# DerekGloudemans/3D-playground

Hardware: AMD Instinct MI355X
Metric: training images/sec at 1920x1080, ResNet-50 3D-RetinaNet (higher is better)
Workload: dtype f32; 1 GPU; resnet50 directional 3D-RetinaNet, 1920x1080 synthetic frames, batch 8 per GPU, 10 GT boxes/image, fp32, fwd+loss+bwd+clip+Adam (BASELINE configs[1]); global_batch=8, parallelism=dp1

## Files before the change

3d-playground_amd/csrc/conv_igemm_mf16.hip:

```cpp
#include <type_traits>

#include "conv_igemm_tile.h"
#include "conv_wgrad_geom.h"

typedef float f32x4a __attribute__((ext_vector_type(4)));

#ifndef RN_MF16_STG
#define RN_MF16_STG 1
#endif
#ifndef RN_MF16_PF
#define RN_MF16_PF 1
#endif
#ifndef RN_MF16_KO
#define RN_MF16_KO 0
#endif

#define RN_SPLIT_MFMA16(ACC, A, B)                                                        \
    do {                                                                                  \
        ACC = __builtin_amdgcn_mfma_f32_16x16x32_bf16((A).l, (B).h, ACC, 0, 0, 0);        \
        ACC = __builtin_amdgcn_mfma_f32_16x16x32_bf16((A).h, (B).l, ACC, 0, 0, 0);        \
        ACC = __builtin_amdgcn_mfma_f32_16x16x32_bf16((A).m, (B).m, ACC, 0, 0, 0);        \
        ACC = __builtin_amdgcn_mfma_f32_16x16x32_bf16((A).m, (B).h, ACC, 0, 0, 0);        \
        ACC = __builtin_amdgcn_mfma_f32_16x16x32_bf16((A).h, (B).m, ACC, 0, 0, 0);        \
        ACC = __builtin_amdgcn_mfma_f32_16x16x32_bf16((A).h, (B).h, ACC, 0, 0, 0);        \
    } while (0)

template <bool GENERAL, bool RAW, int TERMS, bool STG, int WV = 4>
__device__ __forceinline__ void conv_mf16_tile(const rn_conv_desc &d, const float *__restrict__ x, const float *__restrict__ w,
                                               float *__restrict__ y, const float *__restrict__ scale,
                                               const float *__restrict__ shift, const float *__restrict__ add,
                                               const float *__restrict__ mask, const float *__restrict__ add2, const int tile) {
    constexpr int BK = 32, BM = 32 * WV, BN = 128, NSN = BN / 16;
    constexpr int SR = WV == 8 ? 8 : 16;
    constexpr bool HALF = TERMS == 2;
    constexpr int REC = 32 * TERMS, EB = 2 * TERMS;
    constexpr int BPL = BN * 16;
    constexpr int BSTEP = TERMS * BPL;
    constexpr int NBI = TERMS * BN / 16, IB = NBI / WV;
    constexpr int LDT = BN + 4;
    constexpr int LDSF = 2 * BSTEP > WV * SR * LDT ? 2 * BSTEP : WV * SR * LDT;
    static_assert(NBI % WV == 0 && (WV == 4 || WV == 8) && (TERMS == 2 || TERMS == 3), "tile shape");
    __shared__ float lds[LDSF];

    const int tid = threadIdx.x, lane = tid & 63, wave = tid >> 6;
    const int lr = lane & 15, lg = lane >> 4;
    const int wave_u = __builtin_amdgcn_readfirstlane(wave);
    const int ntn = (d.Cout + BN - 1) / BN;
    const int m0 = (tile / ntn) * BM, n0 = (tile % ntn) * BN;
    const int HoWo = d.Ho * d.Wo;
    const int64_t M = (int64_t)d.N * HoWo;
    const int K = d.kh * d.kw * d.Cin;
    const int Kpad = (K + 31) / 32 * 32;
    const int nks = Kpad / BK;

    const int n_first = (int)(m0 / HoWo);
    const int64_t x_floats = ((int64_t)d.N - 1 - n_first) * d.x_batch_stride + (int64_t)d.Hi * d.Wi * d.Cin;
    const __amdgpu_buffer_rsrc_t rs_a = __builtin_amdgcn_make_buffer_rsrc(
        const_cast<float *>(x + (int64_t)n_first * d.x_batch_stride), (short)0,
        (int)(unsigned)(x_floats * 4 > 0x7FFFFFFF ? 0x7FFFFFFF : x_floats * 4), 0x00020000);
    const v4i32 rs_b = make_rsrc(reinterpret_cast<const char *>(w) + (int64_t)n_first * d.w_batch_stride * EB,
                                 (unsigned)((int64_t)d.Cout * Kpad * EB));
    __shared__ float row_unscale[HALF ? BM : 1];
    float a_scale[2] = {1.f, 1.f};

    unsigned a_mask[2];
    int a_base[2];
    int a_n[2] = {-1, -1}, a_rem[2] = {0, 0};
    __shared__ __attribute__((aligned(16))) char a_stage[STG ? WV * Mf16AGeom::WAVE_BYTES : 16];
    __shared__ int4 row_tab[STG ? BM : 1];
    unsigned s_mask[4] = {0u, 0u, 0u, 0u};
    int s_base[4] = {0, 0, 0, 0};
    auto row_geom = [&](int row, unsigned &mk, int &base, int &n_abs, int &rem_) {
        int a_h = -(1 << 28), a_w = 0, a_img = 0;
        n_abs = -1; rem_ = 0;
        if ((int64_t)m0 + row < M) {
            const unsigned rel = (unsigned)(m0 - n_first * HoWo + row);
            const unsigned n = rel / (unsigned)HoWo;
            const unsigned rem = rel - n * (unsigned)HoWo;
            const unsigned oh = rem / (unsigned)d.Wo, ow = rem - oh * (unsigned)d.Wo;
            a_img = (int)((int64_t)n * d.x_batch_stride * 4);
            a_h = (int)oh * d.a + d.p;
            a_w = (int)ow * d.a + d.p_w;
            n_abs = n_first + (int)n; rem_ = (int)rem;
        }
        mk = 0;
        for (int r = 0, t = 0; r < d.kh; ++r)
            for (int s_ = 0; s_ < d.kw; ++s_, ++t) {
                const int ih = a_h + r * d.b, iw = a_w + s_ * d.b;
                mk |= (unsigned)(((ih | iw) >= 0) & (ih < d.Hi) & (iw < d.Wi)) << t;
            }
        base = a_img + (a_h * d.Wi + a_w) * d.Cin * 4;
    };
    if constexpr (STG) {
        if (tid < BM) {
            unsigned mk; int base, n_abs, rem_;
            row_geom(tid, mk, base, n_abs, rem_);
            row_tab[tid] = make_int4(base, (int)mk, n_abs, rem_);
        }
        __syncthreads();
#pragma unroll
        for (int j = 0; j < 4; ++j) {
            const int4 e = row_tab[32 * wave + Mf16AGeom::dma_row(lane, j)];
            s_base[j] = e.x + 16 * Mf16AGeom::dma_chunk(lane, j);
            s_mask[j] = (unsigned)e.y;
        }
#pragma unroll
        for (int sm = 0; sm < 2; ++sm) {
            const int4 e = row_tab[32 * wave + 16 * sm + lr];
            a_n[sm] = e.z; a_rem[sm] = e.w;
            a_mask[sm] = 0u; a_base[sm] = 0;
        }
    } else {
#pragma unroll
        for (int sm = 0; sm < 2; ++sm) {
            row_geom(32 * wave + 16 * sm + lr, a_mask[sm], a_base[sm], a_n[sm], a_rem[sm]);
            a_base[sm] += 8 * lg * 4;
        }
    }
    int f_r = 0, f_s = 0, f_c = 0;
    typedef float f32x4v __attribute__((ext_vector_type(4)));
    struct ARegs { f32x4v v[4]; };
    auto load_a = [&](ARegs &ar) {
#if RN_MF16_KO & 2
        if (f_c >= 0) { f_c += BK; return; }
#endif
        const int t = f_r * d.kw + f_s;
        const int delta = (f_r * d.Wi + f_s) * d.b * d.Cin * 4;
#pragma unroll
        for (int sm = 0; sm < 2; ++sm) {
            const unsigned valid = 0u - ((a_mask[sm] >> (t & 31)) & 1u);
            const unsigned v = ((unsigned)(a_base[sm] + delta) & valid) | (0x80000000u & ~valid);
            ar.v[2 * sm] = __builtin_bit_cast(f32x4v, __builtin_amdgcn_raw_buffer_load_b128(rs_a, (int)v, f_c * 4, 0));
            ar.v[2 * sm + 1] = __builtin_bit_cast(f32x4v, __builtin_amdgcn_raw_buffer_load_b128(rs_a, (int)(v + 16u), f_c * 4, 0));
        }
        f_c += BK;
        const bool wrap = f_c >= d.Cin;
        f_c = wrap ? 0 : f_c;
        f_s += wrap ? 1 : 0;
        const bool wrap_s = f_s == d.kw;
        f_s = wrap_s ? 0 : f_s;
        f_r += wrap_s ? 1 : 0;
    };

    const v4i32 rs_a4 = make_rsrc(x + (int64_t)n_first * d.x_batch_stride, (unsigned)(x_floats * 4 > 0x7FFFFFFF ? 0x7FFFFFFF : x_floats * 4));
    const unsigned a_lds0 = lds_addr(a_stage) + (unsigned)__builtin_amdgcn_readfirstlane(wave) * Mf16AGeom::WAVE_BYTES;
    auto dma_a = [&]() {
#if RN_MF16_KO & 2
        if (f_c >= 0) { f_c += BK; return; }
#endif
        const int t = f_r * d.kw + f_s;
        const int delta = (f_r * d.Wi + f_s) * d.b * d.Cin * 4;
        const unsigned soff = (unsigned)__builtin_amdgcn_readfirstlane(f_c * 4);
#pragma unroll
        for (int j = 0; j < 4; ++j) {
            const unsigned valid = 0u - ((s_mask[j] >> (t & 31)) & 1u);
            dma16(rs_a4, a_lds0 + 1024u * j, ((unsigned)(s_base[j] + delta) & valid) | (0x80000000u & ~valid), soff);
        }
        f_c += BK;
        const bool wrap = f_c >= d.Cin;
        f_c = wrap ? 0 : f_c;
        f_s += wrap ? 1 : 0;
        const bool wrap_s = f_s == d.kw;
        f_s = wrap_s ? 0 : f_s;
        f_r += wrap_s ? 1 : 0;
    };
    const char *a_rd = a_stage + wave * Mf16AGeom::WAVE_BYTES;
    const int a_ra[2][2] = {{Mf16AGeom::read_addr(lane, 0, 0), Mf16AGeom::read_addr(lane, 0, 1)},
                            {Mf16AGeom::read_addr(lane, 1, 0), Mf16AGeom::read_addr(lane, 1, 1)}};
    auto read_a = [&](ARegs &ar) {
#pragma unroll
        for (int sm = 0; sm < 2; ++sm) {
            ar.v[2 * sm] = *reinterpret_cast<const f32x4v *>(a_rd + a_ra[sm][0]);
            ar.v[2 * sm + 1] = *reinterpret_cast<const f32x4v *>(a_rd + a_ra[sm][1]);
        }
    };

    unsigned b_voff[IB];
#pragma unroll
    for (int j = 0; j < IB; ++j) {
        const int q = wave * IB + j, plane = q / (BN / 16), brow = (q % (BN / 16)) * 16 + (lane >> 2);
        const int c = Mf16Geom::dma_chunk(lane);
        const int n = n0 + brow;
        b_voff[j] = n < d.Cout ? (unsigned)(n * Kpad * EB + (c >> 1) * REC + plane * 32 + (c & 1) * 16) : 0x80000000u;
    }
    const unsigned lds0 = lds_addr(lds);
    auto dma_b = [&](int ks, int buf) {
#if RN_MF16_KO & 8
        if (ks > 0) return;
#endif
#pragma unroll
        for (int j = 0; j < IB; ++j)
            dma16(rs_b, lds0 + (unsigned)(buf * BSTEP * 4 + (wave_u * IB + j) * 1024), b_voff[j], (unsigned)(ks * 2 * REC));
    };

    f32x4a acc[2][NSN];
#pragma unroll
    for (int i = 0; i < 2; ++i)
#pragma unroll
        for (int j = 0; j < NSN; ++j) acc[i][j] = f32x4a{0.f, 0.f, 0.f, 0.f};
    const int fb0 = Mf16Geom::read_addr(lane, 0) / 4;

    constexpr int PF = RN_MF16_PF;
    static_assert(!STG || PF == 1, "staged activations: one step in flight");
    ARegs ar[PF] = {};
    if constexpr (STG) dma_a(); else load_a(ar[0]);
    dma_b(0, 0);
#pragma unroll
    for (int i = 1; i < PF; ++i) load_a(ar[i]);
    if constexpr (HALF) {
        int e[2];
        if (d.x_amax_row_stride == 0) {
            const unsigned char *tb = reinterpret_cast<const unsigned char *>(d.x_amax);
            e[0] = rn_amax_exp_lanes(a_n[0] < 0 ? nullptr : tb + (int64_t)a_n[0] * d.x_amax_img_stride * RN_AMAX_BYTES);
            e[1] = __ballot(a_n[1] != a_n[0]) == 0ull ? e[0]
                 : rn_amax_exp_lanes(a_n[1] < 0 ? nullptr : tb + (int64_t)a_n[1] * d.x_amax_img_stride * RN_AMAX_BYTES);
        } else {
#pragma unroll
            for (int sm = 0; sm < 2; ++sm)
                e[sm] = a_n[sm] < 0 ? 0 : (int)((reinterpret_cast<const unsigned *>(d.x_amax)[(int64_t)a_rem[sm] * d.x_amax_row_stride] >> 23) & 0xffu);
        }
#pragma unroll
        for (int sm = 0; sm < 2; ++sm) {
            const int se = rn_f16_scale_exp_of(e[sm]);
            a_scale[sm] = rn_exp_to_float(se);
            if (lg == 0) row_unscale[32 * wave + 16 * sm + lr] = rn_exp_to_float(254 - se);
        }
    }
    constexpr int CPR = BN / 4, RPI = 64 / CPR;
    const int c4 = lane % CPR;
    const int col = n0 + 4 * c4;
    const bool col_ok = col < d.Cout;
    const bool vec = true;
    const int ncol = 4;
    rn_wait_but<4 * (PF - 1)>();
    __syncthreads();
    auto k_step = [&](int ks, int rb, ARegs &cur) {
        if constexpr (STG) read_a(cur);
        asm volatile("" : "+v"(cur.v[0]), "+v"(cur.v[1]), "+v"(cur.v[2]), "+v"(cur.v[3]));
        typename std::conditional<HALF, SplitH8, Split8>::type sa[2];
#if RN_MF16_KO & 1
#pragma unroll
        for (int q = 0; q < 4; ++q) acc[q & 1][q >> 1] += cur.v[q];
        dma_b(ks + 1, rb ^ 1);
        if constexpr (STG) { asm volatile("s_waitcnt lgkmcnt(0)" ::: "memory"); dma_a(); } else load_a(cur);
        rn_wait_dma();
        __syncthreads();
        if (ks >= 0) return;
#endif
#pragma unroll
        for (int sm = 0; sm < 2; ++sm) {
            const float av[8] = {cur.v[2 * sm][0], cur.v[2 * sm][1], cur.v[2 * sm][2], cur.v[2 * sm][3],
                                 cur.v[2 * sm + 1][0], cur.v[2 * sm + 1][1], cur.v[2 * sm + 1][2], cur.v[2 * sm + 1][3]};
            if constexpr (HALF) sa[sm] = split8h(av, a_scale[sm]);
            else sa[sm] = split8(av);
        }
        dma_b(ks + 1, rb ^ 1);
        if constexpr (STG) {
            asm volatile("s_waitcnt lgkmcnt(0)" ::: "memory");
            dma_a();
        } else load_a(cur);
        const float *S = lds + rb * BSTEP + fb0;
#pragma unroll
        for (int sn = 0; sn < NSN; ++sn) {
            if constexpr (HALF) {
                SplitH8 sb;
                sb.h = *reinterpret_cast<const f16x8 *>(S + 256 * sn);
                sb.l = *reinterpret_cast<const f16x8 *>(S + 256 * sn + BPL);
#pragma unroll
                for (int sm = 0; sm < 2; ++sm) RN_SPLITH_MFMA16(acc[sm][sn], sa[sm], sb);
            } else {
                Split8 sb;
                sb.h = *reinterpret_cast<const bf16x8 *>(S + 256 * sn);
                sb.m = *reinterpret_cast<const bf16x8 *>(S + 256 * sn + BPL);
                sb.l = *reinterpret_cast<const bf16x8 *>(S + 256 * sn + 2 * BPL);
#pragma unroll
                for (int sm = 0; sm < 2; ++sm) RN_SPLIT_MFMA16(acc[sm][sn], sa[sm], sb);
            }
        }
        RN_PIN();
        rn_wait_but<4 * (PF - 1)>();
        __syncthreads();
    };
    constexpr int UN = PF > 2 ? PF : 2;
    for (int ks = 0; ks < nks; ks += UN) {
#pragma unroll
        for (int u = 0; u < UN; ++u)
            if (u == 0 || ks + u < nks) k_step(ks + u, u & 1, ar[u % PF]);
    }

    float *T = lds + wave * (SR * LDT);
    float sc[4] = {1.f, 1.f, 1.f, 1.f}, sh[4] = {0.f, 0.f, 0.f, 0.f};
#pragma unroll
    for (int j = 0; j < 4; ++j) {
        if (!RAW && col_ok && scale != nullptr) sc[j] = scale[col + j];
        if (!RAW && col_ok && shift != nullptr) sh[j] = shift[col + j];
        if (HALF && col_ok) sc[j] *= d.w_unscale[(d.w_batch_stride != 0 ? (int64_t)n_first * d.Cout : 0) + col + j];
    }
    float rn_am = 0.f;
    const int64_t m_last = (int64_t)m0 + BM - 1 < M ? (int64_t)m0 + BM - 1 : M - 1;
    const bool rn_span = (int)(m0 / HoWo) != (int)(m_last / HoWo);
#pragma unroll
    for (int smh = 0; smh < 2 * (16 / SR); ++smh) {
        const int sm = smh / (16 / SR), hp = smh % (16 / SR);
        if (SR == 16 || (lg >> 1) == hp) {
#pragma unroll
            for (int sn = 0; sn < NSN; ++sn)
#pragma unroll
                for (int e = 0; e < 4; ++e) T[(4 * lg + e - hp * SR) * LDT + 16 * sn + lr] = acc[sm][sn][e];
        }
        __builtin_amdgcn_fence(__ATOMIC_RELEASE, "wavefront");
        __builtin_amdgcn_wave_barrier();
        __builtin_amdgcn_fence(__ATOMIC_ACQUIRE, "wavefront");
        constexpr int NIT = SR / RPI, G = 4;
        if (col_ok) {
#pragma unroll 1
            for (int g = 0; g < NIT; g += G) {
                int64_t off_[G];
                float4 mk_[G], ad_[G];
#pragma unroll
                for (int i = 0; i < G; ++i) {
                    const int64_t mr = (int64_t)m0 + 32 * wave + 16 * sm + hp * SR + lane / CPR + RPI * (g + i);
                    const int64_t m = mr < M ? mr : M - 1;
                    RN_EPI_ADDR(GENERAL)
                    off_[i] = off;
                    mk_[i] = make_float4(1.f, 1.f, 1.f, 1.f);
                    ad_[i] = make_float4(0.f, 0.f, 0.f, 0.f);
                    if (!RAW && d.mask_mode != 0) mk_[i] = rn_mask_load4(mask, off, (d.mask_mode & RN_MASK_BITS) != 0);
                    if (!RAW && d.add_mode != 0) ad_[i] = *reinterpret_cast<const float4 *>(add + aoff);
                    (void)a2off;
                }
#pragma unroll
                for (int i = 0; i < G; ++i) {
                    const int r = lane / CPR + RPI * (g + i);
                    const int64_t m = (int64_t)m0 + 32 * wave + 16 * sm + hp * SR + r;
                    if (m < M) {
                        float4 t = *reinterpret_cast<const float4 *>(T + r * LDT + 4 * c4);
                        if constexpr (HALF) { const float ru = row_unscale[32 * wave + 16 * sm + hp * SR + r]; t.x *= ru; t.y *= ru; t.z *= ru; t.w *= ru; }
                        const int64_t off = off_[i];
                        float mk[4] = {mk_[i].x, mk_[i].y, mk_[i].z, mk_[i].w}, ad[4] = {ad_[i].x, ad_[i].y, ad_[i].z, ad_[i].w};
                        if (!RAW && d.add2_mode == 3) {
                            int64_t a2;
                            { RN_EPI_ADDR(GENERAL) a2 = a2off; (void)aoff; (void)off; }
                            if (a2 >= 0) { const float4 q = *reinterpret_cast<const float4 *>(add2 + a2); ad[0] += q.x; ad[1] += q.y; ad[2] += q.z; ad[3] += q.w; }
                        }
#if RN_MF16_KO & 4
                        if (t.x != 1.2345f) continue;
#endif
                        if (RAW) *reinterpret_cast<float4 *>(y + off) = HALF ? make_float4(t.x * sc[0], t.y * sc[1], t.z * sc[2], t.w * sc[3]) : t;
                        else { RN_EPI_FINISH() }
                    }
                }
            }
        }
        __builtin_amdgcn_fence(__ATOMIC_RELEASE, "wavefront");
        __builtin_amdgcn_wave_barrier();
    }
    if (!RAW && !rn_span) rn_amax_note(d.y_amax, m0 / HoWo, rn_am);
}

#ifndef RN_MF16H_OCC
#define RN_MF16H_OCC 3
#endif
template <bool GENERAL, bool RAW, int TERMS, bool STG, int WV = 4>
__global__ __launch_bounds__(64 * WV, WV == 8 ? 2 : (TERMS == 2 ? RN_MF16H_OCC : 3)) void conv_igemm_mf16_kernel(const rn_conv_desc d, const float *__restrict__ x,
                                                              const float *__restrict__ w, float *__restrict__ y,
                                                              const float *__restrict__ scale, const float *__restrict__ shift,
                                                              const float *__restrict__ add, const float *__restrict__ mask,
                                                              const float *__restrict__ add2) {
    conv_mf16_tile<GENERAL, RAW, TERMS, STG, WV>(d, x, w, y, scale, shift, add, mask, add2, xcd_remap(blockIdx.x, gridDim.x));
}

template <int TERMS>
__global__ __launch_bounds__(256, TERMS == 2 ? RN_MF16H_OCC : 3) void conv_igemm_mf16_grouped_kernel(const rn_conv_group g, const float *__restrict__ w,
                                                                      const float *__restrict__ scale,
                                                                      const float *__restrict__ shift) {
    const int tile = xcd_remap(blockIdx.x, gridDim.x);
    int p = 0;
#pragma unroll
    for (int i = 0; i < RN_MAX_GROUP - 1; ++i) p += (i + 1 < g.n && tile >= g.tile_end[i]) ? 1 : 0;
    rn_conv_desc d = g.d[0];
    const float *x = g.x[0], *add = g.add[0], *mask = g.mask[0];
    float *y = g.y[0];
    int first = 0;
#pragma unroll
    for (int i = 1; i < RN_MAX_GROUP; ++i)
        if (p == i) { d = g.d[i]; x = g.x[i]; y = g.y[i]; add = g.add[i]; mask = g.mask[i]; first = g.tile_end[i - 1]; }
    conv_mf16_tile<true, false, TERMS, TERMS == 2 && RN_MF16_STG != 0>(d, x, w, y, scale, shift, add, mask, nullptr, tile - first);
}

static int mf16_on() { return rn_get_option(RN_OPT_MF16); }
static int mf16_min_tiles() { return rn_get_option(RN_OPT_MF16_MIN); }
static bool mf16_geom_ok(const rn_conv_desc *d) {
    return (d->Cin % 32) == 0 && d->div_shift == 0 && d->kh * d->kw <= 24 && (d->Cout % 4) == 0 && d->Cout > 64 && !d->in_relu;
}
static bool mf16_ok(const rn_conv_desc *d) {
    if (!mf16_on() || !mf16_geom_ok(d)) return false;
    if (d->w_format == 3) return d->x_amax != nullptr && d->w_unscale != nullptr;
    return d->w_format == 1;
}
static int64_t mf16_tiles(const rn_conv_desc *d) {
    const int64_t M = (int64_t)d->N * d->Ho * d->Wo;
    return ((M + 127) / 128) * ((d->Cout + 127) / 128);
}

extern "C" int rn_conv_igemm_wants_f16(const rn_conv_desc *d) {
    return rn_get_fp32_mfma() == RN_FP32_SPLIT3 && d->w_batch_stride >= 0;
}

bool rn_igemm_mf16_launch(int variant, const rn_conv_desc *d, const float *x, const float *w, float *y, const float *scale,
                          const float *shift, const float *add, const float *mask, const float *add2, hipStream_t s, int *rc) {
    if (!mf16_ok(d) || (variant != 0 && variant != 4 && variant != 5)) return false;
    const int64_t tiles = mf16_tiles(d);
    const int64_t M_rows = (int64_t)d->N * d->Ho * d->Wo;
    if (tiles < mf16_min_tiles() || tiles > 0x7fffffff) return false;
    const dim3 grid((unsigned)tiles), block(256);
#define RN_MF16_LAUNCH(G, R, T, S) hipLaunchKernelGGL((conv_igemm_mf16_kernel<G, R, T, S>), grid, block, 0, s, *d, x, w, y, scale, shift, add, mask, add2)
    if (d->w_format == 3) {
        static const int stg_min_k = [] { const char *e = getenv("RN_MF16_STG_MIN_K"); return e ? atoi(e) : 256; }();
        const bool stg = RN_MF16_STG != 0 && d->kh * d->kw * d->Cin >= stg_min_k;
        static const int wv8_min = [] { const char *e = getenv("RN_MF16_WV8_MIN"); return e ? atoi(e) : 1; }();
        const int64_t tiles8 = ((M_rows + 255) / 256) * ((d->Cout + 127) / 128);
        if (stg && wv8_min > 0 && d->w_batch_stride == 0 && tiles8 >= wv8_min && tiles8 <= 0x7fffffff) {
            const dim3 grid8((unsigned)tiles8), block8(512);
#define RN_MF16_LAUNCH8(G, R) hipLaunchKernelGGL((conv_igemm_mf16_kernel<G, R, 2, true, 8>), grid8, block8, 0, s, *d, x, w, y, scale, shift, add, mask, add2)
            if (variant == 0) RN_MF16_LAUNCH8(false, true);
            else if (variant == 4) RN_MF16_LAUNCH8(false, false);
            else RN_MF16_LAUNCH8(true, false);
#undef RN_MF16_LAUNCH8
        } else
        if (variant == 0) { if (stg) RN_MF16_LAUNCH(false, true, 2, true); else RN_MF16_LAUNCH(false, true, 2, false); }
        else if (variant == 4) { if (stg) RN_MF16_LAUNCH(false, false, 2, true); else RN_MF16_LAUNCH(false, false, 2, false); }
        else { if (stg) RN_MF16_LAUNCH(true, false, 2, true); else RN_MF16_LAUNCH(true, false, 2, false); }
    } else {
        if (variant == 0) RN_MF16_LAUNCH(false, true, 3, false);
        else if (variant == 4) RN_MF16_LAUNCH(false, false, 3, false);
        else RN_MF16_LAUNCH(true, false, 3, false);
    }
#undef RN_MF16_LAUNCH
    const hipError_t e = hipGetLastError();
    *rc = e == hipSuccess ? RN_OK : (int)e;
    return true;
}

bool rn_igemm_mf16_grouped_launch(const rn_conv_group *g, const float *w, const float *scale, const float *shift, hipStream_t s, int *rc) {
    for (int i = 0; i < g->n; ++i)
        if (!mf16_ok(&g->d[i]) || g->d[i].w_format != g->d[0].w_format) return false;
    rn_conv_group gb = *g;
    int64_t total = 0;
    for (int i = 0; i < g->n; ++i) {
        total += mf16_tiles(&g->d[i]);
        gb.tile_end[i] = (int)total;
    }
    for (int i = g->n; i < RN_MAX_GROUP; ++i) gb.tile_end[i] = (int)total;
    if (total < mf16_min_tiles() || total > 0x7fffffff) return false;
    if (g->d[0].w_format == 3) hipLaunchKernelGGL(conv_igemm_mf16_grouped_kernel<2>, dim3((unsigned)total), dim3(256), 0, s, gb, w, scale, shift);
    else hipLaunchKernelGGL(conv_igemm_mf16_grouped_kernel<3>, dim3((unsigned)total), dim3(256), 0, s, gb, w, scale, shift);
    const hipError_t e = hipGetLastError();
    *rc = e == hipSuccess ? RN_OK : (int)e;
    return true;
}
```

3d-playground_amd/csrc/elementwise.hip:

```cpp
#include "common.h"
#include "mfma_split.h"

__global__ void pack_weights_kernel(const float *__restrict__ src, float *__restrict__ dst, int Cout, int Cin, int kh, int kw,
                                    int kw_pad, int c_pad, int mode, const float *__restrict__ scale, int rows, int Kpad,
                                    int r0, int nr, int s0, int ns) {
    const int64_t i = (int64_t)blockIdx.x * 256 + threadIdx.x;
    if (i >= (int64_t)rows * Kpad) return;
    const int row = (int)(i / Kpad), k = (int)(i - (int64_t)row * Kpad);
    const int tap = k / c_pad, c = k - tap * c_pad;
    int r = tap / kw_pad, s = tap - r * kw_pad;
    bool in_filter = r < kh && s < kw;
    if (mode == 2) {
        r = tap / ns;
        s = tap - r * ns;
        in_filter = r < nr;
        r = r0 + 2 * r;
        s = s0 + 2 * s;
    }
    float v = 0.f;
    if (in_filter) {
        if (mode == 0) {
            if (c < Cin) v = src[(((int64_t)row * Cin + c) * kh + r) * kw + s];
        } else {
            if (c < Cout) {
                v = src[(((int64_t)c * Cin + row) * kh + r) * kw + s];
                if (scale) v *= scale[c];
            }
        }
    }
    dst[i] = v;
}

extern "C" int rn_pack_weights(const float *src, float *dst, int Cout, int Cin, int kh, int kw, int kw_pad, int c_pad,
                               int mode, const float *scale, int r0, int nr, int s0, int ns, void *stream) {
    if (Cout <= 0 || Cin <= 0 || kh <= 0 || kw <= 0 || kw_pad < kw || (c_pad & 3) || mode < 0 || mode > 2) return RN_EINVAL;
    if (c_pad < (mode == 0 ? Cin : Cout)) return RN_EINVAL;
    if (mode == 2 && (nr <= 0 || ns <= 0 || r0 < 0 || s0 < 0 || r0 + 2 * (nr - 1) >= kh || s0 + 2 * (ns - 1) >= kw))
        return RN_EINVAL;
    const int rows = mode == 0 ? Cout : Cin;
    const int Kpad = ((mode == 2 ? nr * ns : kh * kw_pad) * c_pad + 31) / 32 * 32;
    hipLaunchKernelGGL(pack_weights_kernel, dim3(rn_blocks((int64_t)rows * Kpad, 256)), dim3(256), 0, (hipStream_t)stream, src,
                       dst, Cout, Cin, kh, kw, kw_pad, c_pad, mode, scale, rows, Kpad, r0, nr, s0, ns);
    RN_LAUNCH_CHECK();
    return RN_OK;
}

__device__ __forceinline__ void unpack_wgrad_channel(const int co, const float *__restrict__ dw, const float *__restrict__ wp,
                                                     float *__restrict__ dweight, int Cin, int kh, int kw, int kw_pad,
                                                     int c_pad, int Kpad, const float *__restrict__ scale,
                                                     const float *__restrict__ mean, const float *__restrict__ rstd,
                                                     const float *__restrict__ colsum, float *__restrict__ dgamma,
                                                     float *__restrict__ dbeta) {
    __shared__ double red[4];
    const float sc = scale ? scale[co] : 1.f;
    const float *row = dw + (int64_t)co * Kpad;
    const float *wrow = wp + (int64_t)co * Kpad;
    const int n = Cin * kh * kw;
    double dot = 0.0;
    for (int i = threadIdx.x; i < n; i += 256) {
        const int ci = i / (kh * kw), rs = i - ci * (kh * kw);
        const int r = rs / kw, s = rs - r * kw;
        const int k = (r * kw_pad + s) * c_pad + ci;
        const float g = row[k];
        dweight[(int64_t)co * n + i] = sc * g;
        if (dgamma) dot += (double)wrow[k] * (double)g;
    }
    if (dgamma) {
        dot = wave_sum(dot);
        if ((threadIdx.x & 63) == 0) red[threadIdx.x >> 6] = dot;
        __syncthreads();
        if (threadIdx.x == 0) {
            const double t = (red[0] + red[1]) + (red[2] + red[3]);
            dgamma[co] = (float)((t - (double)mean[co] * (double)colsum[co]) * (double)rstd[co]);
        }
    }
    if (dbeta && threadIdx.x == 0) dbeta[co] = colsum[co];
}

__global__ __launch_bounds__(256) void unpack_wgrad_kernel(const float *__restrict__ dw, const float *__restrict__ wp,
                                                           float *__restrict__ dweight, int Cin, int kh, int kw, int kw_pad,
                                                           int c_pad, int Kpad, const float *__restrict__ scale,
                                                           const float *__restrict__ mean, const float *__restrict__ rstd,
                                                           const float *__restrict__ colsum, float *__restrict__ dgamma,
                                                           float *__restrict__ dbeta) {
    unpack_wgrad_channel(blockIdx.x, dw, wp, dweight, Cin, kh, kw, kw_pad, c_pad, Kpad, scale, mean, rstd, colsum, dgamma, dbeta);
}

__global__ __launch_bounds__(256) void unpack_batched_kernel(const rn_unpack_job *__restrict__ jobs, const int2 *__restrict__ chunks) {
    const int2 c = chunks[blockIdx.x];
    const rn_unpack_job j = jobs[c.x];
    unpack_wgrad_channel(c.y, j.dw, j.w_packed, j.dweight, j.Cin, j.kh, j.kw, j.kw_pad, j.c_pad, j.Kpad, j.scale, j.mean, j.rstd,
                         j.colsum, j.dgamma, j.dbeta);
}

extern "C" int rn_unpack_batched(const rn_unpack_job *jobs_dev, const int32_t *chunks_dev, int nchunks, void *stream) {
    if (!jobs_dev || !chunks_dev || nchunks <= 0) return RN_EINVAL;
    hipLaunchKernelGGL(unpack_batched_kernel, dim3(nchunks), dim3(256), 0, (hipStream_t)stream, jobs_dev,
                       reinterpret_cast<const int2 *>(chunks_dev));
    RN_LAUNCH_CHECK();
    return RN_OK;
}

extern "C" int rn_unpack_wgrad(const float *dw, const float *w_packed, float *dweight, int Cout, int Cin, int kh, int kw,
                               int kw_pad, int c_pad, const float *scale, const float *mean, const float *rstd,
                               const float *colsum, float *dgamma, float *dbeta, void *stream) {
    if (Cout <= 0 || Cin <= 0 || kw_pad < kw || c_pad < Cin) return RN_EINVAL;
    if ((dgamma || dbeta) && !colsum) return RN_EINVAL;
    if (dgamma && (!mean || !rstd || !w_packed)) return RN_EINVAL;
    const int Kpad = (kh * kw_pad * c_pad + 31) / 32 * 32;
    hipLaunchKernelGGL(unpack_wgrad_kernel, dim3(Cout), dim3(256), 0, (hipStream_t)stream, dw, w_packed, dweight, Cin, kh, kw,
                       kw_pad, c_pad, Kpad, scale, mean, rstd, colsum, dgamma, dbeta);
    RN_LAUNCH_CHECK();
    return RN_OK;
}

__global__ void bn_fold_kernel(const float *__restrict__ gamma, const float *__restrict__ beta, const float *__restrict__ mean,
                               const float *__restrict__ var, float eps, int C, float *__restrict__ scale,
                               float *__restrict__ shift, float *__restrict__ rstd) {
    const int c = blockIdx.x * 256 + threadIdx.x;
    if (c >= C) return;
    const float rs = 1.0f / sqrtf(var[c] + eps);
    const float s = gamma[c] * rs;
    scale[c] = s;
    shift[c] = beta[c] - mean[c] * s;
    if (rstd) rstd[c] = rs;
}

extern "C" int rn_bn_fold(const float *gamma, const float *beta, const float *mean, const float *var, float eps, int C,
                          float *scale, float *shift, float *rstd, void *stream) {
    if (C <= 0) return RN_EINVAL;
    hipLaunchKernelGGL(bn_fold_kernel, dim3(rn_blocks(C, 256)), dim3(256), 0, (hipStream_t)stream, gamma, beta, mean, var, eps,
                       C, scale, shift, rstd);
    RN_LAUNCH_CHECK();
    return RN_OK;
}

__global__ __launch_bounds__(256) void prep_batched_kernel(const rn_prep_job *__restrict__ jobs, const int2 *__restrict__ chunks) {
    const int2 c = chunks[blockIdx.x];
    const rn_prep_job j = jobs[c.x];
    const int64_t i = (int64_t)c.y * 256 + threadIdx.x;
    if (j.kind == 0) {
        if (i >= j.Cout) return;
        const float rs = 1.0f / sqrtf(j.var[i] + j.eps);
        const float sc = j.gamma[i] * rs;
        j.bn_scale[i] = sc;
        j.bn_shift[i] = j.beta[i] - j.mean[i] * sc;
        j.bn_rstd[i] = rs;
        return;
    }
    if (j.kind == 5) {
        const int64_t row = (int64_t)c.y * 4 + (threadIdx.x >> 6);
        if (row < j.rows) split_row_f16(j.src, j.dst, j.bn_scale, row, j.Kpad, threadIdx.x & 63);
        return;
    }
    if (j.kind == 4) {
        if (i < (int64_t)j.rows * j.Kpad / 8) split_store_chunk(j.src, j.dst, i);
        return;
    }
    if (i >= (int64_t)j.rows * j.Kpad) return;
    if (j.kind == 3) {
        reinterpret_cast<__bf16 *>(j.dst)[i] = (__bf16)j.src[i];
        return;
    }
    if (j.kind == 2) {
        const int row = (int)(i / j.Kpad), k = (int)(i - (int64_t)row * j.Kpad);
        const int kdim = j.mode == 0 ? j.Cin : j.Cout;
        float g[3][3];
#pragma unroll
        for (int r = 0; r < 3; ++r)
#pragma unroll
            for (int s = 0; s < 3; ++s) {
                float v = 0.f;
                if (k < kdim) {
                    if (j.mode == 0) v = j.src[(((int64_t)row * j.Cin + k) * 3 + r) * 3 + s];
                    else v = j.src[(((int64_t)k * j.Cin + row) * 3 + (2 - r)) * 3 + (2 - s)] * (j.scale ? j.scale[k] : 1.f);
                }
                g[r][s] = v;
            }
        float t[6][3];
#pragma unroll
        for (int s = 0; s < 3; ++s) {
            const float a = g[0][s], b = g[1][s], c = g[2][s];
            t[0][s] = a * (1.f / 4.f);
            t[1][s] = -(a + b + c) * (1.f / 6.f);
            t[2][s] = (b - a - c) * (1.f / 6.f);
            t[3][s] = a * (1.f / 24.f) + b * (1.f / 12.f) + c * (1.f / 6.f);
            t[4][s] = a * (1.f / 24.f) - b * (1.f / 12.f) + c * (1.f / 6.f);
            t[5][s] = c;
        }
#pragma unroll
        for (int a6i = 0; a6i < 6; ++a6i) {
            const float a = t[a6i][0], b = t[a6i][1], c = t[a6i][2];
            const float o[6] = {a * (1.f / 4.f), -(a + b + c) * (1.f / 6.f), (b - a - c) * (1.f / 6.f),
                                a * (1.f / 24.f) + b * (1.f / 12.f) + c * (1.f / 6.f),
                                a * (1.f / 24.f) - b * (1.f / 12.f) + c * (1.f / 6.f), c};
#pragma unroll
            for (int b6 = 0; b6 < 6; ++b6) j.dst[((int64_t)(a6i * 6 + b6) * j.rows + row) * j.Kpad + k] = o[b6];
        }
        return;
    }
    const int row = (int)(i / j.Kpad), k = (int)(i - (int64_t)row * j.Kpad);
    const int tap = k / j.c_pad, ch = k - tap * j.c_pad;
    int r = tap / j.kw_pad, s = tap - r * j.kw_pad;
    bool in_filter = r < j.kh && s < j.kw;
    if (j.mode == 2) {
        r = tap / j.ns;
        s = tap - r * j.ns;
        in_filter = r < j.nr;
        r = j.r0 + 2 * r;
        s = j.s0 + 2 * s;
    }
    float v = 0.f;
    if (in_filter) {
        if (j.mode == 0) {
            if (ch < j.Cin) v = j.src[(((int64_t)row * j.Cin + ch) * j.kh + r) * j.kw + s];
        } else if (ch < j.Cout) {
            v = j.src[(((int64_t)ch * j.Cin + row) * j.kh + r) * j.kw + s];
            if (j.scale) v *= j.scale[ch];
        }
    }
    j.dst[i] = v;
}

extern "C" int rn_prep_batched(const rn_prep_job *jobs_dev, const int32_t *chunks_dev, int nchunks, void *stream) {
    if (!jobs_dev || !chunks_dev || nchunks <= 0) return RN_EINVAL;
    hipLaunchKernelGGL(prep_batched_kernel, dim3(nchunks), dim3(256), 0, (hipStream_t)stream, jobs_dev,
                       reinterpret_cast<const int2 *>(chunks_dev));
    RN_LAUNCH_CHECK();
    return RN_OK;
}

__global__ void nchw_to_nhwc4_kernel(const float *__restrict__ src, float4 *__restrict__ dst, int64_t HW, int64_t total, unsigned *__restrict__ amax) {
    const int64_t i = (int64_t)blockIdx.x * 256 + threadIdx.x;
    if (i >= total) return;
    const int64_t n = i / HW, p = i - n * HW;
    const float *s = src + n * 3 * HW + p;
    const float4 v = make_float4(s[0], s[HW], s[2 * HW], 0.f);
    dst[i] = v;
    rn_amax_note(amax, n, fmaxf(fmaxf(fabsf(v.x), fabsf(v.y)), fabsf(v.z)));
}

extern "C" int rn_nchw_to_nhwc4(const float *src, float *dst, int N, int H, int W, void *amax, void *stream) {
    if (N <= 0 || H <= 0 || W <= 0) return RN_EINVAL;
    const int64_t HW = (int64_t)H * W, total = HW * N;
    hipLaunchKernelGGL(nchw_to_nhwc4_kernel, dim3(rn_blocks(total, 256)), dim3(256), 0, (hipStream_t)stream, src,
                       reinterpret_cast<float4 *>(dst), HW, total, reinterpret_cast<unsigned *>(amax));
    RN_LAUNCH_CHECK();
    return RN_OK;
}

__global__ void maxpool_fwd_kernel(const float4 *__restrict__ x, float4 *__restrict__ y, uchar4 *__restrict__ arg, int H, int W,
                                   int C4, int Ho, int Wo, int64_t total) {
    const int64_t i = (int64_t)xcd_remap(blockIdx.x, gridDim.x) * 256 + threadIdx.x;
    if (i >= total) return;
    const int c = (int)(i % C4);
    int64_t t = i / C4;
    const int ow = (int)(t % Wo);
    t /= Wo;
    const int oh = (int)(t % Ho);
    const int64_t n = t / Ho;
    float4 m = make_float4(-INFINITY, -INFINITY, -INFINITY, -INFINITY);
    uchar4 a = make_uchar4(0, 0, 0, 0);
#pragma unroll
    for (int r = 0; r < 3; ++r) {
        const int ih = oh * 2 - 1 + r;
        if ((unsigned)ih >= (unsigned)H) continue;
#pragma unroll
        for (int s = 0; s < 3; ++s) {
            const int iw = ow * 2 - 1 + s;
            if ((unsigned)iw >= (unsigned)W) continue;
            const float4 v = x[((n * H + ih) * W + iw) * C4 + c];
            const unsigned char pos = (unsigned char)(3 * r + s);
            if (v.x > m.x) { m.x = v.x; a.x = pos; }
            if (v.y > m.y) { m.y = v.y; a.y = pos; }
            if (v.z > m.z) { m.z = v.z; a.z = pos; }
            if (v.w > m.w) { m.w = v.w; a.w = pos; }
        }
    }
    y[i] = m;
    if (arg) arg[i] = a;
}

extern "C" int rn_maxpool_fwd(const float *x, float *y, uint8_t *argmax, int N, int H, int W, int C, int Ho, int Wo,
                              void *stream) {
    if (N <= 0 || (C & 3) || Ho != (H + 2 - 3) / 2 + 1 || Wo != (W + 2 - 3) / 2 + 1) return RN_EINVAL;
    const int64_t total = (int64_t)N * Ho * Wo * (C / 4);
    hipLaunchKernelGGL(maxpool_fwd_kernel, dim3(rn_blocks(total, 256)), dim3(256), 0, (hipStream_t)stream,
                       reinterpret_cast<const float4 *>(x), reinterpret_cast<float4 *>(y), reinterpret_cast<uchar4 *>(argmax), H,
                       W, C / 4, Ho, Wo, total);
    RN_LAUNCH_CHECK();
    return RN_OK;
}

__global__ void maxpool_bwd_kernel(const float4 *__restrict__ x, const float4 *__restrict__ dy, const uchar4 *__restrict__ arg,
                                   float4 *__restrict__ dx, int H, int W, int C4, int Ho, int Wo, int relu_mask, int64_t total,
                                   unsigned *__restrict__ amax) {
    const int64_t i = (int64_t)xcd_remap(blockIdx.x, gridDim.x) * 256 + threadIdx.x;
    if (i >= total) return;
    const int c = (int)(i % C4);
    int64_t t = i / C4;
    const int iw = (int)(t % W);
    t /= W;
    const int ih = (int)(t % H);
    const int64_t n = t / H;
    float4 g = make_float4(0.f, 0.f, 0.f, 0.f);
    for (int oh = ih / 2; oh <= (ih + 1) / 2; ++oh) {
        if (oh >= Ho) continue;
        const int r = ih - (oh * 2 - 1);
        for (int ow = iw / 2; ow <= (iw + 1) / 2; ++ow) {
            if (ow >= Wo) continue;
            const unsigned char pos = (unsigned char)(3 * r + (iw - (ow * 2 - 1)));
            const int64_t o = ((n * Ho + oh) * Wo + ow) * C4 + c;
            const uchar4 a = arg[o];
            const float4 d = dy[o];
            if (a.x == pos) g.x += d.x;
            if (a.y == pos) g.y += d.y;
            if (a.z == pos) g.z += d.z;
            if (a.w == pos) g.w += d.w;
        }
    }
    if (relu_mask) {
        const float4 v = rn_mask_load4(reinterpret_cast<const float *>(x), 4 * i, relu_mask == 2);
        g.x = v.x > 0.f ? g.x : 0.f; g.y = v.y > 0.f ? g.y : 0.f; g.z = v.z > 0.f ? g.z : 0.f; g.w = v.w > 0.f ? g.w : 0.f;
    }
    dx[i] = g;
    rn_amax_note(amax, n, fmaxf(fmaxf(fabsf(g.x), fabsf(g.y)), fmaxf(fabsf(g.z), fabsf(g.w))));
}

extern "C" int rn_maxpool_bwd(const float *x, const float *dy, const uint8_t *argmax, float *dx, int N, int H, int W, int C,
                              int Ho, int Wo, int relu_mask, void *amax, void *stream) {
    if (N <= 0 || (C & 3) || argmax == nullptr || Ho != (H + 2 - 3) / 2 + 1 || Wo != (W + 2 - 3) / 2 + 1) return RN_EINVAL;
    if (relu_mask < 0 || relu_mask > 2 || (relu_mask == 2 && (C & 31))) return RN_EINVAL;
    const int64_t total = (int64_t)N * H * W * (C / 4);
    hipLaunchKernelGGL(maxpool_bwd_kernel, dim3(rn_blocks(total, 256)), dim3(256), 0, (hipStream_t)stream,
                       reinterpret_cast<const float4 *>(x), reinterpret_cast<const float4 *>(dy),
                       reinterpret_cast<const uchar4 *>(argmax), reinterpret_cast<float4 *>(dx), H, W, C / 4, Ho, Wo, relu_mask,
                       total, reinterpret_cast<unsigned *>(amax));
    RN_LAUNCH_CHECK();
    return RN_OK;
}

#define CS_ROWS 512
extern "C" int64_t rn_colsum_workspace_bytes(int64_t rows, int C) {
    return ((rows + CS_ROWS - 1) / CS_ROWS) * (int64_t)C * sizeof(float);
}

__global__ __launch_bounds__(256) void colsum_partial_kernel(const float *__restrict__ g, int64_t rows, int C, int ld,
                                                             float *__restrict__ part) {
    const int c = blockIdx.y * 256 + threadIdx.x;
    if (c >= C) return;
    const int64_t r0 = (int64_t)blockIdx.x * CS_ROWS;
    const int64_t r1 = r0 + CS_ROWS < rows ? r0 + CS_ROWS : rows;
    float s0 = 0.f, s1 = 0.f, s2 = 0.f, s3 = 0.f;
    int64_t r = r0;
    for (; r + 3 < r1; r += 4) {
        s0 += g[r * ld + c]; s1 += g[(r + 1) * ld + c]; s2 += g[(r + 2) * ld + c]; s3 += g[(r + 3) * ld + c];
    }
    for (; r < r1; ++r) s0 += g[r * ld + c];
    part[(int64_t)blockIdx.x * C + c] = (s0 + s1) + (s2 + s3);
}
__global__ __launch_bounds__(256) void colsum_final_kernel(const float *__restrict__ part, int64_t nchunks, int C,
                                                           float *__restrict__ out, int accumulate) {
    const int c = blockIdx.x * 256 + threadIdx.x;
    if (c >= C) return;
    double s = accumulate ? (double)out[c] : 0.0;
    for (int64_t k = 0; k < nchunks; ++k) s += part[k * C + c];
    out[c] = (float)s;
}

extern "C" int rn_colsum(const float *g, int64_t rows, int C, int ld, float *out, int accumulate, void *workspace,
                         void *stream) {
    if (rows <= 0 || C <= 0 || ld < C) return RN_EINVAL;
    const int64_t nchunks = (rows + CS_ROWS - 1) / CS_ROWS;
    float *part = reinterpret_cast<float *>(workspace);
    hipLaunchKernelGGL(colsum_partial_kernel, dim3((unsigned)nchunks, (C + 255) / 256), dim3(256), 0, (hipStream_t)stream, g,
                       rows, C, ld, part);
    hipLaunchKernelGGL(colsum_final_kernel, dim3((C + 255) / 256), dim3(256), 0, (hipStream_t)stream, (const float *)part,
                       nchunks, C, out, accumulate);
    RN_LAUNCH_CHECK();
    return RN_OK;
}

__global__ void upsample_add_bwd_kernel(const float4 *__restrict__ src, float4 *__restrict__ dst, int Hs, int Ws, int Hd, int Wd,
                                        int C4, int64_t total, unsigned *__restrict__ amax) {
    const int64_t i = (int64_t)blockIdx.x * 256 + threadIdx.x;
    if (i >= total) return;
    const int c = (int)(i % C4);
    int64_t t = i / C4;
    const int w = (int)(t % Wd);
    t /= Wd;
    const int h = (int)(t % Hd);
    const int64_t n = t / Hd;
    float4 a = dst[i];
#pragma unroll
    for (int dy = 0; dy < 2; ++dy) {
        const int hs = 2 * h + dy;
        if (hs >= Hs) continue;
#pragma unroll
        for (int dx = 0; dx < 2; ++dx) {
            const int ws = 2 * w + dx;
            if (ws >= Ws) continue;
            const float4 v = src[((n * Hs + hs) * Ws + ws) * C4 + c];
            a.x += v.x; a.y += v.y; a.z += v.z; a.w += v.w;
        }
    }
    dst[i] = a;
    rn_amax_note(amax, n, fmaxf(fmaxf(fabsf(a.x), fabsf(a.y)), fmaxf(fabsf(a.z), fabsf(a.w))));
}

extern "C" int rn_upsample_add_bwd(const float *src, float *dst, int N, int Hs, int Ws, int Hd, int Wd, int C, void *amax, void *stream) {
    if (N <= 0 || (C & 3)) return RN_EINVAL;
    const int64_t total = (int64_t)N * Hd * Wd * (C / 4);
    hipLaunchKernelGGL(upsample_add_bwd_kernel, dim3(rn_blocks(total, 256)), dim3(256), 0, (hipStream_t)stream,
                       reinterpret_cast<const float4 *>(src), reinterpret_cast<float4 *>(dst), Hs, Ws, Hd, Wd, C / 4, total,
                       reinterpret_cast<unsigned *>(amax));
    RN_LAUNCH_CHECK();
    return RN_OK;
}

__global__ void relu_mask_kernel(float *__restrict__ g, const float *__restrict__ z, int64_t n) {
    const int64_t i = (int64_t)blockIdx.x * 256 + threadIdx.x;
    if (i < n) g[i] = z[i] > 0.f ? g[i] : 0.f;
}
extern "C" int rn_relu_mask(float *g, const float *z, int64_t n, void *stream) {
    if (n <= 0) return RN_EINVAL;
    hipLaunchKernelGGL(relu_mask_kernel, dim3(rn_blocks(n, 256)), dim3(256), 0, (hipStream_t)stream, g, z, n);
    RN_LAUNCH_CHECK();
    return RN_OK;
}

__global__ void sigmoid_bwd_pad_kernel(const float *__restrict__ dy, const float *__restrict__ s, float *__restrict__ out,
                                       int64_t rows, int64_t rpi, int C, int ld, int64_t bstride, unsigned *__restrict__ amax) {
    const int64_t i = (int64_t)blockIdx.x * 256 + threadIdx.x;
    if (i >= rows * ld) return;
    const int64_t r = i / ld;
    const int c = (int)(i - r * ld);
    const int64_t b = r / rpi;
    float v = 0.f;
    if (c < C) {
        const int64_t src = b * bstride + (r - b * rpi) * C + c;
        v = dy[src];
        if (s) { const float p = s[src]; v *= p * (1.0f - p); }
    }
    out[i] = v;
    rn_amax_note(amax, b, fabsf(v));
}
extern "C" int rn_sigmoid_bwd_pad(const float *dy, const float *s, float *out, int B, int64_t rows_per_image, int C, int ld,
                                  int64_t src_batch_stride, void *amax, void *stream) {
    const int64_t rows = (int64_t)B * rows_per_image;
    if (rows <= 0 || C <= 0 || ld < C) return RN_EINVAL;
    hipLaunchKernelGGL(sigmoid_bwd_pad_kernel, dim3(rn_blocks(rows * ld, 256)), dim3(256), 0, (hipStream_t)stream, dy, s, out,
                       rows, rows_per_image, C, ld, src_batch_stride, reinterpret_cast<unsigned *>(amax));
    RN_LAUNCH_CHECK();
    return RN_OK;
}

__global__ void add_inplace_kernel(float *__restrict__ dst, const float *__restrict__ src, int64_t n, int64_t per_image, unsigned *__restrict__ amax) {
    const int64_t i = (int64_t)blockIdx.x * 256 + threadIdx.x;
    if (i >= n) return;
    const int64_t img = amax != nullptr ? i / per_image : 0;
    const float v = dst[i] + src[i];
    dst[i] = v;
    rn_amax_note(amax, img, fabsf(v));
}
extern "C" int rn_add_inplace(float *dst, const float *src, int64_t n, int64_t per_image, void *amax, void *stream) {
    if (n <= 0 || (amax != nullptr && per_image <= 0)) return RN_EINVAL;
    hipLaunchKernelGGL(add_inplace_kernel, dim3(rn_blocks(n, 256)), dim3(256), 0, (hipStream_t)stream, dst, src, n, per_image,
                       reinterpret_cast<unsigned *>(amax));
    RN_LAUNCH_CHECK();
    return RN_OK;
}
```

Before: 124.3 images/sec.

## Add 64-column MFMA conv tile for narrow convs and restructure maxpool backward

Convolutions with at most 64 output channels can now use the split-bf16 MFMA implicit-GEMM path through a new 8-wave, 64-column tile instead of falling back to a slower kernel. This is aimed at layers such as the ResNet stem and the early 64-channel bottlenecks. Separately, maxpool backward now gives each thread one 2x2 input block, so each argmax/dy entry is loaded once and shared across up to four outputs. It also indexes with 32-bit integers when the element count fits. Together these reduce redundant gathers and integer division cost, at the price of a new kernel instantiation whose tile efficiency with 64 columns is unproven.

```diff
diff --git a/3d-playground_amd/csrc/conv_igemm_mf16.hip b/3d-playground_amd/csrc/conv_igemm_mf16.hip
--- a/3d-playground_amd/csrc/conv_igemm_mf16.hip
+++ b/3d-playground_amd/csrc/conv_igemm_mf16.hip
@@ -25,12 +25,12 @@
         ACC = __builtin_amdgcn_mfma_f32_16x16x32_bf16((A).h, (B).h, ACC, 0, 0, 0);        \
     } while (0)
 
-template <bool GENERAL, bool RAW, int TERMS, bool STG, int WV = 4>
+template <bool GENERAL, bool RAW, int TERMS, bool STG, int WV = 4, int BN = 128>
 __device__ __forceinline__ void conv_mf16_tile(const rn_conv_desc &d, const float *__restrict__ x, const float *__restrict__ w,
                                                float *__restrict__ y, const float *__restrict__ scale,
                                                const float *__restrict__ shift, const float *__restrict__ add,
                                                const float *__restrict__ mask, const float *__restrict__ add2, const int tile) {
-    constexpr int BK = 32, BM = 32 * WV, BN = 128, NSN = BN / 16;
+    constexpr int BK = 32, BM = 32 * WV, NSN = BN / 16;
     constexpr int SR = WV == 8 ? 8 : 16;
     constexpr bool HALF = TERMS == 2;
     constexpr int REC = 32 * TERMS, EB = 2 * TERMS;
@@ -39,7 +39,9 @@
     constexpr int NBI = TERMS * BN / 16, IB = NBI / WV;
     constexpr int LDT = BN + 4;
     constexpr int LDSF = 2 * BSTEP > WV * SR * LDT ? 2 * BSTEP : WV * SR * LDT;
-    static_assert(NBI % WV == 0 && (WV == 4 || WV == 8) && (TERMS == 2 || TERMS == 3), "tile shape");
+    static_assert(NBI % WV == 0 && IB >= 1 && (WV == 4 || WV == 8) && (TERMS == 2 || TERMS == 3), "tile shape");
+    static_assert(BN == 128 || (BN == 64 && WV == 8 && TERMS == 2 && !RAW), "the 64-column form: eight waves, fp16 terms, never the plain GEMM");
+    static_assert(64 % (BN / 4) == 0 && SR % (64 / (BN / 4)) == 0, "epilogue: whole strip rows per wave instruction, whole instructions per strip");
     __shared__ float lds[LDSF];
 
     const int tid = threadIdx.x, lane = tid & 63, wave = tid >> 6;
@@ -311,7 +313,8 @@
         __builtin_amdgcn_fence(__ATOMIC_RELEASE, "wavefront");
         __builtin_amdgcn_wave_barrier();
         __builtin_amdgcn_fence(__ATOMIC_ACQUIRE, "wavefront");
-        constexpr int NIT = SR / RPI, G = 4;
+        constexpr int NIT = SR / RPI, G = NIT < 4 ? NIT : 4;
+        static_assert(NIT % G == 0, "epilogue strip");
         if (col_ok) {
 #pragma unroll 1
             for (int g = 0; g < NIT; g += G) {
@@ -361,13 +364,13 @@
 #ifndef RN_MF16H_OCC
 #define RN_MF16H_OCC 3
 #endif
-template <bool GENERAL, bool RAW, int TERMS, bool STG, int WV = 4>
+template <bool GENERAL, bool RAW, int TERMS, bool STG, int WV = 4, int BN = 128>
 __global__ __launch_bounds__(64 * WV, WV == 8 ? 2 : (TERMS == 2 ? RN_MF16H_OCC : 3)) void conv_igemm_mf16_kernel(const rn_conv_desc d, const float *__restrict__ x,
                                                               const float *__restrict__ w, float *__restrict__ y,
                                                               const float *__restrict__ scale, const float *__restrict__ shift,
                                                               const float *__restrict__ add, const float *__restrict__ mask,
                                                               const float *__restrict__ add2) {
-    conv_mf16_tile<GENERAL, RAW, TERMS, STG, WV>(d, x, w, y, scale, shift, add, mask, add2, xcd_remap(blockIdx.x, gridDim.x));
+    conv_mf16_tile<GENERAL, RAW, TERMS, STG, WV, BN>(d, x, w, y, scale, shift, add, mask, add2, xcd_remap(blockIdx.x, gridDim.x));
 }
 
 template <int TERMS>
@@ -390,8 +393,12 @@
 
 static int mf16_on() { return rn_get_option(RN_OPT_MF16); }
 static int mf16_min_tiles() { return rn_get_option(RN_OPT_MF16_MIN); }
+static bool mf16_n64(const rn_conv_desc *d) {
+    static const int on = [] { const char *e = getenv("RN_MF16_N64"); return e ? atoi(e) : 1; }();
+    return d->Cout <= 64 && on != 0 && d->w_format == 3 && d->w_batch_stride == 0;
+}
 static bool mf16_geom_ok(const rn_conv_desc *d) {
-    return (d->Cin % 32) == 0 && d->div_shift == 0 && d->kh * d->kw <= 24 && (d->Cout % 4) == 0 && d->Cout > 64 && !d->in_relu;
+    return (d->Cin % 32) == 0 && d->div_shift == 0 && d->kh * d->kw <= 24 && (d->Cout % 4) == 0 && (d->Cout > 64 || mf16_n64(d)) && !d->in_relu;
 }
 static bool mf16_ok(const rn_conv_desc *d) {
     if (!mf16_on() || !mf16_geom_ok(d)) return false;
@@ -400,6 +407,7 @@
 }
 static int64_t mf16_tiles(const rn_conv_desc *d) {
     const int64_t M = (int64_t)d->N * d->Ho * d->Wo;
+    if (d->Cout <= 64) return (M + 255) / 256;
     return ((M + 127) / 128) * ((d->Cout + 127) / 128);
 }
 
@@ -409,7 +417,9 @@
 
 bool rn_igemm_mf16_launch(int variant, const rn_conv_desc *d, const float *x, const float *w, float *y, const float *scale,
                           const float *shift, const float *add, const float *mask, const float *add2, hipStream_t s, int *rc) {
-    if (!mf16_ok(d) || (variant != 0 && variant != 4 && variant != 5)) return false;
+    if (!mf16_ok(d)) return false;
+    const bool n64 = d->Cout <= 64;
+    if (n64 ? (variant != 2 && variant != 3) : (variant != 0 && variant != 4 && variant != 5)) return false;
     const int64_t tiles = mf16_tiles(d);
     const int64_t M_rows = (int64_t)d->N * d->Ho * d->Wo;
     if (tiles < mf16_min_tiles() || tiles > 0x7fffffff) return false;
@@ -420,6 +430,13 @@
         const bool stg = RN_MF16_STG != 0 && d->kh * d->kw * d->Cin >= stg_min_k;
         static const int wv8_min = [] { const char *e = getenv("RN_MF16_WV8_MIN"); return e ? atoi(e) : 1; }();
         const int64_t tiles8 = ((M_rows + 255) / 256) * ((d->Cout + 127) / 128);
+        if (n64) {
+            const dim3 grid64((unsigned)tiles), block64(512);
+#define RN_MF16_LAUNCH64(G, S) hipLaunchKernelGGL((conv_igemm_mf16_kernel<G, false, 2, S, 8, 64>), grid64, block64, 0, s, *d, x, w, y, scale, shift, add, mask, add2)
+            if (variant == 2) { if (stg) RN_MF16_LAUNCH64(false, true); else RN_MF16_LAUNCH64(false, false); }
+            else { if (stg) RN_MF16_LAUNCH64(true, true); else RN_MF16_LAUNCH64(true, false); }
+#undef RN_MF16_LAUNCH64
+        } else
         if (stg && wv8_min > 0 && d->w_batch_stride == 0 && tiles8 >= wv8_min && tiles8 <= 0x7fffffff) {
             const dim3 grid8((unsigned)tiles8), block8(512);
 #define RN_MF16_LAUNCH8(G, R) hipLaunchKernelGGL((conv_igemm_mf16_kernel<G, R, 2, true, 8>), grid8, block8, 0, s, *d, x, w, y, scale, shift, add, mask, add2)
@@ -444,7 +461,7 @@
 
 bool rn_igemm_mf16_grouped_launch(const rn_conv_group *g, const float *w, const float *scale, const float *shift, hipStream_t s, int *rc) {
     for (int i = 0; i < g->n; ++i)
-        if (!mf16_ok(&g->d[i]) || g->d[i].w_format != g->d[0].w_format) return false;
+        if (!mf16_ok(&g->d[i]) || g->d[i].w_format != g->d[0].w_format || g->d[i].Cout <= 64) return false;
     rn_conv_group gb = *g;
     int64_t total = 0;
     for (int i = 0; i < g->n; ++i) {
diff --git a/3d-playground_amd/csrc/elementwise.hip b/3d-playground_amd/csrc/elementwise.hip
--- a/3d-playground_amd/csrc/elementwise.hip
+++ b/3d-playground_amd/csrc/elementwise.hip
@@ -292,50 +292,95 @@
     return RN_OK;
 }
 
-__global__ void maxpool_bwd_kernel(const float4 *__restrict__ x, const float4 *__restrict__ dy, const uchar4 *__restrict__ arg,
-                                   float4 *__restrict__ dx, int H, int W, int C4, int Ho, int Wo, int relu_mask, int64_t total,
-                                   unsigned *__restrict__ amax) {
-    const int64_t i = (int64_t)xcd_remap(blockIdx.x, gridDim.x) * 256 + threadIdx.x;
-    if (i >= total) return;
-    const int c = (int)(i % C4);
-    int64_t t = i / C4;
-    const int iw = (int)(t % W);
-    t /= W;
-    const int ih = (int)(t % H);
-    const int64_t n = t / H;
-    float4 g = make_float4(0.f, 0.f, 0.f, 0.f);
-    for (int oh = ih / 2; oh <= (ih + 1) / 2; ++oh) {
-        if (oh >= Ho) continue;
-        const int r = ih - (oh * 2 - 1);
-        for (int ow = iw / 2; ow <= (iw + 1) / 2; ++ow) {
-            if (ow >= Wo) continue;
-            const unsigned char pos = (unsigned char)(3 * r + (iw - (ow * 2 - 1)));
-            const int64_t o = ((n * Ho + oh) * Wo + ow) * C4 + c;
-            const uchar4 a = arg[o];
-            const float4 d = dy[o];
-            if (a.x == pos) g.x += d.x;
-            if (a.y == pos) g.y += d.y;
-            if (a.z == pos) g.z += d.z;
-            if (a.w == pos) g.w += d.w;
-        }
-    }
+template <typename IT>
+__global__ __launch_bounds__(256) void maxpool_bwd_kernel(const float4 *__restrict__ x, const float4 *__restrict__ dy,
+                                                          const uchar4 *__restrict__ arg, float4 *__restrict__ dx, int H, int W, int C4,
+                                                          int Ho, int Wo, int Hb, int Wb, int relu_mask, int64_t total,
+                                                          unsigned *__restrict__ amax) {
+    const int64_t i64 = (int64_t)xcd_remap(blockIdx.x, gridDim.x) * 256 + threadIdx.x;
+    if (i64 >= total) return;
+    const IT i = (IT)i64;
+    const int c = (int)(i % (IT)C4);
+    IT t = i / (IT)C4;
+    const int bw = (int)(t % (IT)Wb);
+    t /= (IT)Wb;
+    const int bh = (int)(t % (IT)Hb);
+    const int64_t n = (int64_t)(t / (IT)Hb);
+    const bool wB = bw + 1 < Wo, wC = bh + 1 < Ho;
+    const bool pR = 2 * bh + 1 < H, pC = 2 * bw + 1 < W;
+    const int64_t oA = ((n * Ho + bh) * Wo + bw) * C4 + c, oC = oA + (int64_t)Wo * C4;
+    const float4 z4 = make_float4(0.f, 0.f, 0.f, 0.f);
+    const uchar4 none = make_uchar4(255, 255, 255, 255);
+    const uchar4 aA = arg[oA];
+    const float4 dA = dy[oA];
+    const uchar4 aB = wB && pC ? arg[oA + C4] : none;
+    const float4 dB = wB && pC ? dy[oA + C4] : z4;
+    const uchar4 aC = wC && pR ? arg[oC] : none;
+    const float4 dC = wC && pR ? dy[oC] : z4;
+    const uchar4 aD = wB && wC && pR && pC ? arg[oC + C4] : none;
+    const float4 dD = wB && wC && pR && pC ? dy[oC + C4] : z4;
+    const int64_t p00 = ((n * H + 2 * bh) * W + 2 * bw) * C4 + c, p10 = p00 + (int64_t)W * C4;
+    float4 m00 = make_float4(1.f, 1.f, 1.f, 1.f), m01 = m00, m10 = m00, m11 = m00;
     if (relu_mask) {
-        const float4 v = rn_mask_load4(reinterpret_cast<const float *>(x), 4 * i, relu_mask == 2);
-        g.x = v.x > 0.f ? g.x : 0.f; g.y = v.y > 0.f ? g.y : 0.f; g.z = v.z > 0.f ? g.z : 0.f; g.w = v.w > 0.f ? g.w : 0.f;
-    }
-    dx[i] = g;
-    rn_amax_note(amax, n, fmaxf(fmaxf(fabsf(g.x), fabsf(g.y)), fmaxf(fabsf(g.z), fabsf(g.w))));
+        const float *xm = reinterpret_cast<const float *>(x);
+        m00 = rn_mask_load4(xm, 4 * p00, relu_mask == 2);
+        if (pC) m01 = rn_mask_load4(xm, 4 * (p00 + C4), relu_mask == 2);
+        if (pR) m10 = rn_mask_load4(xm, 4 * p10, relu_mask == 2);
+        if (pR && pC) m11 = rn_mask_load4(xm, 4 * (p10 + C4), relu_mask == 2);
+    }
+    float am = 0.f;
+#define RN_POOL_TAKE(A, D, POS)                \
+    if (A.x == POS) g.x += D.x;                \
+    if (A.y == POS) g.y += D.y;                \
+    if (A.z == POS) g.z += D.z;                \
+    if (A.w == POS) g.w += D.w;
+#define RN_POOL_STORE(OFF, M)                                                                                           \
+    g.x = M.x > 0.f ? g.x : 0.f; g.y = M.y > 0.f ? g.y : 0.f; g.z = M.z > 0.f ? g.z : 0.f; g.w = M.w > 0.f ? g.w : 0.f; \
+    dx[OFF] = g;                                                                                                        \
+    am = fmaxf(am, fmaxf(fmaxf(fabsf(g.x), fabsf(g.y)), fmaxf(fabsf(g.z), fabsf(g.w))));
+    {
+        float4 g = z4;
+        RN_POOL_TAKE(aA, dA, 4)
+        RN_POOL_STORE(p00, m00)
+    }
+    if (pC) {
+        float4 g = z4;
+        RN_POOL_TAKE(aA, dA, 5)
+        RN_POOL_TAKE(aB, dB, 3)
+        RN_POOL_STORE(p00 + C4, m01)
+    }
+    if (pR) {
+        float4 g = z4;
+        RN_POOL_TAKE(aA, dA, 7)
+        RN_POOL_TAKE(aC, dC, 1)
+        RN_POOL_STORE(p10, m10)
+    }
+    if (pR && pC) {
+        float4 g = z4;
+        RN_POOL_TAKE(aA, dA, 8)
+        RN_POOL_TAKE(aB, dB, 6)
+        RN_POOL_TAKE(aC, dC, 2)
+        RN_POOL_TAKE(aD, dD, 0)
+        RN_POOL_STORE(p10 + C4, m11)
+    }
+#undef RN_POOL_TAKE
+#undef RN_POOL_STORE
+    rn_amax_note(amax, n, am);
 }
 
 extern "C" int rn_maxpool_bwd(const float *x, const float *dy, const uint8_t *argmax, float *dx, int N, int H, int W, int C,
                               int Ho, int Wo, int relu_mask, void *amax, void *stream) {
     if (N <= 0 || (C & 3) || argmax == nullptr || Ho != (H + 2 - 3) / 2 + 1 || Wo != (W + 2 - 3) / 2 + 1) return RN_EINVAL;
     if (relu_mask < 0 || relu_mask > 2 || (relu_mask == 2 && (C & 31))) return RN_EINVAL;
-    const int64_t total = (int64_t)N * H * W * (C / 4);
-    hipLaunchKernelGGL(maxpool_bwd_kernel, dim3(rn_blocks(total, 256)), dim3(256), 0, (hipStream_t)stream,
-                       reinterpret_cast<const float4 *>(x), reinterpret_cast<const float4 *>(dy),
-                       reinterpret_cast<const uchar4 *>(argmax), reinterpret_cast<float4 *>(dx), H, W, C / 4, Ho, Wo, relu_mask,
-                       total, reinterpret_cast<unsigned *>(amax));
+    const int Hb = (H + 1) / 2, Wb = (W + 1) / 2;
+    const int64_t total = (int64_t)N * Hb * Wb * (C / 4);
+#define RN_POOL_BWD(IT)                                                                                                             \
+    hipLaunchKernelGGL(maxpool_bwd_kernel<IT>, dim3(rn_blocks(total, 256)), dim3(256), 0, (hipStream_t)stream,                      \
+                       reinterpret_cast<const float4 *>(x), reinterpret_cast<const float4 *>(dy),                                   \
+                       reinterpret_cast<const uchar4 *>(argmax), reinterpret_cast<float4 *>(dx), H, W, C / 4, Ho, Wo, Hb, Wb,       \
+                       relu_mask, total, reinterpret_cast<unsigned *>(amax))
+    if (total <= 0x7fffffffLL) RN_POOL_BWD(unsigned); else RN_POOL_BWD(int64_t);
+#undef RN_POOL_BWD
     RN_LAUNCH_CHECK();
     return RN_OK;
 }
```

Result: no change. 125.2 images/sec (median of 6 runs) (+0.8%).
